# Image-Processing-Systems-Laboratory/DeepInPainting

Hardware: AMD Instinct MI355X
Metric: train images/sec at 256x256, batch 8/GPU, 1/2/4/8 MI355X; IPSR layer ms (higher is better)
Workload: dtype f32; 1 GPU; BASELINE config 2: 256x256 synthetic images, 128x128 centre mask (M=256 of N=1024 feature positions), batch 8/GPU, fp32, full IPSR training step; global_batch=8, parallelism=dp1, dropout=True, conv_math=fp32, vgg16=seeded random init (no pretrained weights offline)

## Files before the change

deepinpainting_amd/csrc/winograd.hip:

```cpp
#include <type_traits>

#include "ipsr_common.h"

namespace ipsr {

typedef float f32x16 __attribute__((ext_vector_type(16)));
typedef const __attribute__((address_space(1))) void* gptr_t;
typedef __attribute__((address_space(3))) void* lptr_t;

constexpr int WG_BM = 128, WG_BN = 128, WG_BK = 16, WG_NBUF = 4, WG_THREADS = 256;

struct WinoSplit {
    int nsplit, sps, xi_split, nsplit_t, sps_t;
    int nxi = 36;
    __host__ __device__ int slabs() const { return xi_split >= nxi ? nsplit : (xi_split <= 0 ? nsplit_t : (nsplit > nsplit_t ? nsplit : nsplit_t)); }
    __host__ __device__ int of(int xi) const { return xi < xi_split ? nsplit : nsplit_t; }
    __host__ __device__ int head_xi() const { return xi_split < nxi ? xi_split : nxi; }
    __host__ int workgroups(int tiles_per_xi) const { return tiles_per_xi * (head_xi() * nsplit + (nxi - head_xi()) * nsplit_t); }
};

__device__ __forceinline__ void wino_load_sum(const float* __restrict__ M, const WinoSplit sp, size_t plane, size_t off, float m[6][6])
{
#pragma unroll
    for (int i = 0; i < 6; ++i)
// ... 1321 lines not shown
            if (oy < Ho && ox < Wo) st1(yp, (size_t)oy * Wo + ox, o[i][j]);
        }
}

constexpr int W5R_TILES = 64;
template <typename TOUT>
__global__ void __launch_bounds__(256) wino5_output_rows_kernel(const float* __restrict__ Mo, WinoSplit split, int B, int K, int Kp, int nh, int nw,
                                                                int TY, int TX, int Tp, TOUT* __restrict__ y)
{
    __shared__ float blk[W5R_TILES][101];
    __shared__ int org_y[W5R_TILES], org_x[W5R_TILES], org_b[W5R_TILES];
    const int tl = threadIdx.x & 63, ph = threadIdx.x >> 6, ey = ph >> 1, ex = ph & 1;
    const int t0 = blockIdx.x * W5R_TILES, t = t0 + tl, k = blockIdx.y;
    const int T = B * TY * TX;
    if (t < T) {
        float m[6][6], o[5][5];
        wino_load_sum(Mo, split, (size_t)Kp * Tp, (size_t)(ph * K + k) * Tp + t, m);
        wino_at5_2d(m, o);
#pragma unroll
        for (int i = 0; i < 5; ++i)
#pragma unroll
            for (int j = 0; j < 5; ++j) blk[tl][(2 * i - ey + 1) * 10 + (2 * j - ex + 1)] = o[i][j];
        if (ph == 0) {
            const int b = t / (TY * TX), rem = t - b * TY * TX;
            const int ty = rem / TX, tx = rem - ty * TX;
            org_b[tl] = b; org_y[tl] = 10 * ty - 1; org_x[tl] = 10 * tx - 1;
        }
    }
    __syncthreads();
    const int Hy = 2 * nh, Wy = 2 * nw;
    const int ntile = min(W5R_TILES, T - t0);
    for (int e = threadIdx.x; e < 10 * 10 * W5R_TILES; e += 256) {
        const int r = e / (10 * W5R_TILES), xs = e - r * (10 * W5R_TILES);
        const int tile = xs / 10, c = xs - tile * 10;
        if (tile >= ntile) continue;
        const int fy = org_y[tile] + r, fx = org_x[tile] + c;
        if (fy < 0 || fy >= Hy || fx < 0 || fx >= Wy) continue;
        st1(y + ((size_t)org_b[tile] * K + k) * (size_t)Hy * Wy, (size_t)fy * Wy + fx, blk[tile][r * 10 + c]);
    }
}

template <int MODE, typename TIN>
__global__ void __launch_bounds__(256) wino_wrw_tile5_kernel(const TIN* __restrict__ dy, int B, int K, int Ho, int Wo, int TY, int TX,
                                                             int Tp, int Kp, void* __restrict__ Et)
{
    __shared__ __attribute__((aligned(16))) unsigned char smem[op_smem_bytes<true, MODE>()];
    const OpIdx ix = op_index<true, MODE>(false);
    const int t = ix.t, k = ix.c, T = B * TY * TX;
    const bool live = t < T && k < K;
    int b = 0, ty = 0, tx = 0;
    if (live) { b = t / (TY * TX); const int rem = t - b * TY * TX; ty = rem / TX; tx = rem - ty * TX; }
    const TIN* dp = dy + ((size_t)b * K + (live ? k : 0)) * Ho * Wo;
    float e[5][5];
#pragma unroll
    for (int i = 0; i < 5; ++i)
#pragma unroll
        for (int j = 0; j < 5; ++j) {
            const int yy = 5 * ty + i, xx = 5 * tx + j;
            e[i][j] = (live && yy < Ho && xx < Wo) ? ld1(dp, (size_t)yy * Wo + xx) : 0.0f;
        }
    float w[6][5], v[6][6];
#pragma unroll
    for (int j = 0; j < 5; ++j) {
        const float col[5] = {e[0][j], e[1][j], e[2][j], e[3][j], e[4][j]};
        float o[6];
        wino_g5(col, o);
#pragma unroll
        for (int i = 0; i < 6; ++i) w[i][j] = o[i];
    }
#pragma unroll
    for (int i = 0; i < 6; ++i) wino_g5(w[i], v[i]);
    op_emit<true, MODE>(smem, v, ix, Et, Kp, Tp);
}

__global__ void __launch_bounds__(256) wino_wrw_output2_kernel(const float* __restrict__ Mw, WinoSplit split, int Kc, int Cf, int Kp, int Cp,
                                                               float* __restrict__ dW)
{
    const int cf = blockIdx.x * 256 + threadIdx.x, kc = blockIdx.y, ph = blockIdx.z;
    if (cf >= Cf) return;
    float m[6][6], w[2][6], o[2][2];
    wino_load_sum(Mw, split, (size_t)Kp * Cp, (size_t)kc * Cp + (size_t)ph * Cf + cf, m);
#pragma unroll
    for (int j = 0; j < 6; ++j) {
        const float col[6] = {m[0][j], m[1][j], m[2][j], m[3][j], m[4][j], m[5][j]};
        float r2[2];
        wino_at2(col, r2);
        w[0][j] = r2[0]; w[1][j] = r2[1];
    }
    wino_at2(w[0], o[0]);
    wino_at2(w[1], o[1]);
    const int ey = ph >> 1, ex = ph & 1;
    float* dst = dW + ((size_t)kc * Cf + cf) * 16;
#pragma unroll
    for (int a = 0; a < 2; ++a)
#pragma unroll
        for (int b = 0; b < 2; ++b) dst[(2 * a + ey) * 4 + 2 * b + ex] = o[a][b];
}

struct S2Plan { int TY, TX, T, Tp, Kp, Cp, red; WinoSplit sp; size_t a_floats, b_floats, m_floats, total_bytes; };

static int s2_plan(int mode, int B, int Kc, int Cf, int nh, int nw, S2Plan* p, int math)
{
    if (mode < 0 || mode > 2) return fail(IPSR_ERR_INVALID, "4x4 stride-2 winograd: mode %d", mode);
    p->TY = mode == 1 ? (nh + 5) / 5 : (nh + 4) / 5;
    p->TX = mode == 1 ? (nw + 5) / 5 : (nw + 4) / 5;
    p->T = B * p->TY * p->TX;
    p->Tp = (p->T + WG_BN - 1) / WG_BN * WG_BN;
    size_t m1;
    if (mode == 2) {
        p->Kp = wino_rows_padded(Kc, math);
        p->Cp = (4 * Cf + WG_BN - 1) / WG_BN * WG_BN;
        p->red = p->Tp;
        p->a_floats = (size_t)36 * p->Tp * p->Kp * 3 / 2;
        p->b_floats = (size_t)36 * p->Tp * p->Cp * 3 / 2;
        m1 = (size_t)36 * p->Kp * p->Cp;
        p->sp = wino_choose_split(36 * wino_row_tiles(p->Kp) * (p->Cp / WG_BN), p->Tp / WG_BK, m1 * 4);
    } else {
        p->red = mode == 0 ? 4 * Cf : Kc;
        if (p->red % WG_BK != 0)
            return fail(IPSR_ERR_UNSUPPORTED, "4x4 stride-2 winograd: reduction length %d is not a multiple of %d", p->red, WG_BK);
        const int prod = mode == 0 ? Kc : 4 * Cf;
        p->Kp = wino_rows_padded(prod, math);
        p->Cp = p->red;
        p->a_floats = (size_t)36 * p->red * p->Kp * 3 / 2;
        p->b_floats = (size_t)36 * p->red * p->Tp * 3 / 2;
        m1 = (size_t)36 * p->Kp * p->Tp;
        p->sp = wino_choose_split(36 * wino_row_tiles(p->Kp) * (p->Tp / WG_BN), p->red / WG_BK, m1 * 4);
    }
    p->m_floats = m1 * p->sp.slabs();
    p->total_bytes = align_up(p->a_floats * 4, 256) + align_up(p->b_floats * 4, 256) + align_up(p->m_floats * 4, 256) + 256;
    return IPSR_OK;
}

size_t winograd_s2_ws_bytes(int mode, int B, int Kc, int Cf, int nh, int nw)
{
    S2Plan p, q;
    if (s2_plan(mode, B, Kc, Cf, nh, nw, &p, -1) != IPSR_OK || s2_plan(mode, B, Kc, Cf, nh, nw, &q, 0) != IPSR_OK) return 0;
    return p.total_bytes > q.total_bytes ? p.total_bytes : q.total_bytes;
}

int launch_winograd_s2(int mode, const void* a, const void* b2, void* out, int B, int Kc, int Cf, int nh, int nw,
                       void* ws, size_t ws_bytes, hipStream_t st, ConvArith ar = ConvArith{0, false, false})
{
    S2Plan p;
    if (int rc = s2_plan(mode, B, Kc, Cf, nh, nw, &p, ar.math)) return rc;
    if (ws_bytes < p.total_bytes) return fail(IPSR_ERR_WORKSPACE, "4x4 stride-2 winograd: workspace %zu < %zu", ws_bytes, p.total_bytes);
    if (!arith_ok(ar)) return fail(IPSR_ERR_INVALID, "4x4 stride-2 winograd: arithmetic %d", ar.math);
    if (ar.math && ((mode == 0 && Cf % 8 != 0) || (mode == 1 && (Cf % SPLIT_ROWS != 0 || p.Kp != 4 * Cf || Kc % 8 != 0)))) ar.math = 0;
    Carver cv(ws, ws_bytes);
    float* A = cv.take<float>(p.a_floats);
    float* Bv = cv.take<float>(p.b_floats);
    float* Mo = cv.take<float>(p.m_floats);
    const int remap = !debug_option(1);
    if (mode == 0 || mode == 1) {
        const float* w = static_cast<const float*>(b2);
        if (ar.math == 0) {
            if (mode == 0) wino52_filter_kernel<<<dim3(cdiv(p.Kp, 256), Cf), 256, 0, st>>>(w, Kc, Cf, p.Kp, 0, A);
            else wino52_filter_kernel<<<dim3(cdiv(Cf + (p.Kp - 4 * Cf), 256), Kc), 256, 0, st>>>(w, Kc, Cf, p.Kp, 1, A);
        } else {
            const dim3 fg = mode == 0 ? dim3(p.Kp / SPLIT_ROWS, Cf / 8) : dim3(Cf / SPLIT_ROWS, Kc / 8);
            if (ar.math == 2) wino52_filter_split_kernel<2><<<fg, 256, 0, st>>>(w, Kc, Cf, p.Kp, mode, reinterpret_cast<unsigned short*>(A));
            else wino52_filter_split_kernel<3><<<fg, 256, 0, st>>>(w, Kc, Cf, p.Kp, mode, reinterpret_cast<unsigned short*>(A));
        }
        with_mode(ar.math, [&](auto M) {
            constexpr int MODE = decltype(M)::value;
            with_type(ar.in_bf16, [&](auto* tag) {
                using T = ELEM_T(tag);
                if (mode == 0) wino5_window_kernel<2, false, MODE, T><<<op_grid(false, MODE, p.Tp, p.red), 256, 0, st>>>(static_cast<const T*>(a), B, Cf, 2 * nh, 2 * nw, 4, p.TY, p.TX, p.Tp, 0, Bv, remap);
                else wino5_window_kernel<1, false, MODE, T><<<op_grid(false, MODE, p.Tp, p.red), 256, 0, st>>>(static_cast<const T*>(a), B, Kc, nh, nw, 1, p.TY, p.TX, p.Tp, 0, Bv, remap);
            });
        });
        if (int rc = check_launch("wino5_window_kernel")) return rc;
        launch_wino_gemm(ar.math, A, Bv, p.red, p.Kp, p.Tp, p.sp, Mo, st, 72.0 * p.red * (mode == 0 ? Kc : 4 * Cf) * p.T);
        if (int rc = check_launch("wino_gemm_kernel")) return rc;
        with_type(ar.out_bf16, [&](auto* tag) {
            using T = ELEM_T(tag);
            if (mode == 0) wino5_output_kernel<T><<<dim3(cdiv(p.T, 256), Kc), 256, 0, st>>>(Mo, p.sp, B, Kc, p.Kp, nh, nw, p.TY, p.TX, p.Tp, static_cast<T*>(out));
            else wino5_output_rows_kernel<T><<<dim3(cdiv(p.T, W5R_TILES), Cf), 256, 0, st>>>(Mo, p.sp, B, Cf, p.Kp, nh, nw, p.TY, p.TX, p.Tp, static_cast<T*>(out));
        });
        return check_launch("wino5_output_kernel");
    }
    with_mode(ar.math, [&](auto M) {
        constexpr int MODE = decltype(M)::value;
        with_type(ar.in_bf16, [&](auto* tag) {
            using T = ELEM_T(tag);
            wino_wrw_tile5_kernel<MODE, T><<<op_grid(true, MODE, p.Tp, p.Kp), 256, 0, st>>>(static_cast<const T*>(b2), B, Kc, nh, nw, p.TY, p.TX, p.Tp, p.Kp, A);
            wino5_window_kernel<2, true, MODE, T><<<op_grid(true, MODE, p.Tp, p.Cp), 256, 0, st>>>(static_cast<const T*>(a), B, Cf, 2 * nh, 2 * nw, 4, p.TY, p.TX, p.Tp, p.Cp, Bv, 0);
        });
    });
    if (int rc = check_launch("wino5_window_kernel")) return rc;
    launch_wino_gemm(ar.math, A, Bv, p.Tp, p.Kp, p.Cp, p.sp, Mo, st, 72.0 * p.T * Kc * 4 * Cf);
    if (int rc = check_launch("wino_gemm_kernel")) return rc;
    wino_wrw_output2_kernel<<<dim3(cdiv(Cf, 256), Kc, 4), 256, 0, st>>>(Mo, p.sp, Kc, Cf, p.Kp, p.Cp, static_cast<float*>(out));
    return check_launch("wino_wrw_output2_kernel");
}

typedef float f32x4v __attribute__((ext_vector_type(4)));


__global__ void __launch_bounds__(256) sm_to_cn_kernel(const float* __restrict__ x, int B, int C, int HW, int Tp, float* __restrict__ out)
{
    const int n = blockIdx.x * 256 + threadIdx.x, c = blockIdx.y;
    if (n >= Tp) return;
    float v = 0.0f;
    if (n < B * HW) { const int b = n / HW, p = n - b * HW; v = x[((size_t)b * C + c) * HW + p]; }
    out[(size_t)c * Tp + n] = v;
}

__global__ void __launch_bounds__(256) sm_to_nc_kernel(const float* __restrict__ x, int B, int C, int HW, float* __restrict__ out)
{
    const int c = blockIdx.x * 256 + threadIdx.x, n = blockIdx.y;
    if (c >= C) return;
    float v = 0.0f;
    if (n < B * HW) { const int b = n / HW, p = n - b * HW; v = x[((size_t)b * C + c) * HW + p]; }
    out[(size_t)n * C + c] = v;
}

__device__ __forceinline__ float sm_tap(const float* __restrict__ f, int B, int C, int Hf, int Wf, int Ho, int Wo, int k, int st, int pad, int dil,
                                        int n, int col)
{
    if (n >= B * Ho * Wo) return 0.0f;
    const int kk = k * k;
    const int c = col / kk, t = col - c * kk, r = t / k, q = t - r * k;
    const int b = n / (Ho * Wo), o = n - b * Ho * Wo, oy = o / Wo, ox = o - oy * Wo;
    const int fy = oy * st - pad + r * dil, fx = ox * st - pad + q * dil;
    return ((unsigned)fy < (unsigned)Hf && (unsigned)fx < (unsigned)Wf) ? f[(((size_t)b * C + c) * Hf + fy) * Wf + fx] : 0.0f;
}

__global__ void __launch_bounds__(256) sm_im2col_nt_kernel(const float* __restrict__ f, int B, int C, int Hf, int Wf, int Ho, int Wo,
                                                           int k, int st, int pad, int dil, float* __restrict__ out)
{
    const int col = blockIdx.x * 256 + threadIdx.x, n = blockIdx.y;
    const int ncol = C * k * k;
    if (col >= ncol) return;
    out[(size_t)n * ncol + col] = sm_tap(f, B, C, Hf, Wf, Ho, Wo, k, st, pad, dil, n, col);
}

__global__ void __launch_bounds__(256) sm_im2col_cn_kernel(const float* __restrict__ f, int B, int C, int Hf, int Wf, int Ho, int Wo,
                                                           int k, int st, int pad, int dil, int Tp, float* __restrict__ out)
{
    const int n = blockIdx.x * 256 + threadIdx.x, col = blockIdx.y;
    if (n >= Tp) return;
    out[(size_t)col * Tp + n] = sm_tap(f, B, C, Hf, Wf, Ho, Wo, k, st, pad, dil, n, col);
}

__global__ void __launch_bounds__(256) sm_col2im_kernel(const float* __restrict__ M, int nslab, size_t slab_stride, int B, int C, int Hf, int Wf,
                                                        int Ho, int Wo, int k, int st, int pad, int dil, int Tp, float* __restrict__ out)
{
    const size_t idx = (size_t)blockIdx.x * 256 + threadIdx.x;
    const size_t total = (size_t)B * C * Hf * Wf;
    if (idx >= total) return;
    const int fx = (int)(idx % Wf), fy = (int)((idx / Wf) % Hf), c = (int)((idx / ((size_t)Wf * Hf)) % C), b = (int)(idx / ((size_t)Wf * Hf * C));
    float acc = 0.0f;
    for (int r = 0; r < k; ++r) {
        const int ny = fy + pad - r * dil;
        if (ny < 0 || ny % st) continue;
        const int oy = ny / st;
        if (oy >= Ho) continue;
        for (int q = 0; q < k; ++q) {
            const int nx = fx + pad - q * dil;
            if (nx < 0 || nx % st) continue;
            const int ox = nx / st;
            if (ox >= Wo) continue;
            const size_t off = (size_t)(c * k * k + r * k + q) * Tp + ((size_t)b * Ho + oy) * Wo + ox;
            for (int sl = 0; sl < nslab; ++sl) acc += M[(size_t)sl * slab_stride + off];
        }
    }
    out[idx] = acc;
}

__global__ void __launch_bounds__(256) sm_sum_to_nchw_kernel(const float* __restrict__ Y, int nslab, size_t slab_stride, int B, int R, int HW, int Tp,
                                                             float* __restrict__ out)
{
    const size_t idx = (size_t)blockIdx.x * 256 + threadIdx.x;
    if (idx >= (size_t)B * R * HW) return;
    const int o = (int)(idx % HW), r = (int)((idx / HW) % R), b = (int)(idx / ((size_t)HW * R));
    const size_t off = (size_t)r * Tp + (size_t)b * HW + o;
    float acc = 0.0f;
    for (int sl = 0; sl < nslab; ++sl) acc += Y[(size_t)sl * slab_stride + off];
    out[idx] = acc;
}

template <int NB>
__device__ __forceinline__ void sm_reduce4(f32x16 (&acc)[NB], float* lds, int wave, int lane)
{
    if (wave > 0) {
#pragma unroll
        for (int nb = 0; nb < NB; ++nb)
#pragma unroll
            for (int e = 0; e < 16; ++e) lds[(((wave - 1) * NB + nb) * 16 + e) * 64 + lane] = acc[nb][e];
    }
    __syncthreads();
    if (wave == 0) {
#pragma unroll
        for (int w = 0; w < 3; ++w)
#pragma unroll
            for (int nb = 0; nb < NB; ++nb)
#pragma unroll
                for (int e = 0; e < 16; ++e) acc[nb][e] += lds[((w * NB + nb) * 16 + e) * 64 + lane];
    }
    __syncthreads();
}

template <int NB>
__global__ void __launch_bounds__(256) sm_data_kernel(const float* __restrict__ Wm, const float* __restrict__ In, int R, int Q, int Tp, int rows_per_wave,
                                                      float* __restrict__ Mcol)
{
    __shared__ float red[3 * NB * 16 * 64];
    const int lane = threadIdx.x & 63, wave = __builtin_amdgcn_readfirstlane(threadIdx.x >> 6), m = lane & 31, h = lane >> 5;
    const int q0 = blockIdx.x * 128, n0 = blockIdx.z * (32 * NB);
    const int ra = min(R, (blockIdx.y * 4 + wave) * rows_per_wave), rb = min(R, ra + rows_per_wave);
    f32x16 acc[4][NB];
#pragma unroll
    for (int j = 0; j < 4; ++j)
#pragma unroll
        for (int nb = 0; nb < NB; ++nb)
#pragma unroll
            for (int e = 0; e < 16; ++e) acc[j][nb][e] = 0.0f;
    const float* wp = Wm + (size_t)(ra + h) * Q + q0 + 4 * m;
    const float* ip = In + (size_t)(ra + h) * Tp + n0 + m;
    constexpr int U = NB == 1 ? 8 : (NB == 2 ? 4 : 2);
    for (int r = ra; r < rb; r += 2 * U) {
        f32x4v a[U];
        float bv[U][NB];
#pragma unroll
        for (int u = 0; u < U; ++u) {
            const bool ok = r + 2 * u < rb;
            a[u] = ok ? *reinterpret_cast<const f32x4v*>(wp + (size_t)2 * u * Q) : f32x4v{0.0f, 0.0f, 0.0f, 0.0f};
#pragma unroll
            for (int nb = 0; nb < NB; ++nb) bv[u][nb] = ok ? ip[(size_t)2 * u * Tp + 32 * nb] : 0.0f;
        }
#pragma unroll
        for (int u = 0; u < U; ++u)
#pragma unroll
            for (int j = 0; j < 4; ++j)
#pragma unroll
                for (int nb = 0; nb < NB; ++nb) acc[j][nb] = __builtin_amdgcn_mfma_f32_32x32x2f32(a[u][j], bv[u][nb], acc[j][nb], 0, 0, 0);
        wp += (size_t)2 * U * Q;
        ip += (size_t)2 * U * Tp;
    }
    float* out = Mcol + (size_t)blockIdx.y * Q * Tp;
#pragma unroll
    for (int j = 0; j < 4; ++j) {
        sm_reduce4<NB>(acc[j], red, wave, lane);
        if (wave == 0) {
#pragma unroll
            for (int nb = 0; nb < NB; ++nb)
#pragma unroll
                for (int e = 0; e < 16; ++e) {
                    const int row = (e & 3) + 8 * (e >> 2) + 4 * h;
                    out[(size_t)(q0 + 4 * row + j) * Tp + n0 + 32 * nb + m] = acc[j][nb][e];
                }
        }
    }
}

template <int NB>
__global__ void __launch_bounds__(256) sm_fwd_kernel(const float* __restrict__ Wm, const float* __restrict__ Xc, int R, int Q, int Tp, int cols_per_wave,
                                                     float* __restrict__ Y)
{
    __shared__ float red[3 * NB * 16 * 64];
    const int lane = threadIdx.x & 63, wave = __builtin_amdgcn_readfirstlane(threadIdx.x >> 6), m = lane & 31, h = lane >> 5;
    const int r0 = blockIdx.x * 32, n0 = blockIdx.z * (32 * NB);
    const int qa = min(Q, (blockIdx.y * 4 + wave) * cols_per_wave), qb = min(Q, qa + cols_per_wave);
    f32x16 acc[NB];
#pragma unroll
    for (int nb = 0; nb < NB; ++nb)
#pragma unroll
        for (int e = 0; e < 16; ++e) acc[nb][e] = 0.0f;
    const float* wp = Wm + (size_t)(r0 + m) * Q + qa + 4 * h;
    const float* xp = Xc + (size_t)(qa + 4 * h) * Tp + n0 + m;
    constexpr int U = 4;
    for (int q = qa; q < qb; q += 8 * U) {
        f32x4v a[U];
        float bv[U][4][NB];
#pragma unroll
        for (int u = 0; u < U; ++u) {
            const bool ok = q + 8 * u < qb;
            a[u] = ok ? *reinterpret_cast<const f32x4v*>(wp + 8 * u) : f32x4v{0.0f, 0.0f, 0.0f, 0.0f};
#pragma unroll
            for (int j = 0; j < 4; ++j)
#pragma unroll
                for (int nb = 0; nb < NB; ++nb) bv[u][j][nb] = ok ? xp[(size_t)(8 * u + j) * Tp + 32 * nb] : 0.0f;
        }
#pragma unroll
        for (int u = 0; u < U; ++u)
#pragma unroll
            for (int j = 0; j < 4; ++j)
#pragma unroll
                for (int nb = 0; nb < NB; ++nb) acc[nb] = __builtin_amdgcn_mfma_f32_32x32x2f32(a[u][j], bv[u][j][nb], acc[nb], 0, 0, 0);
        wp += 8 * U;
        xp += (size_t)8 * U * Tp;
    }
    sm_reduce4<NB>(acc, red, wave, lane);
    if (wave == 0) {
        float* out = Y + (size_t)blockIdx.y * R * Tp;
#pragma unroll
        for (int nb = 0; nb < NB; ++nb)
#pragma unroll
            for (int e = 0; e < 16; ++e) {
                const int row = (e & 3) + 8 * (e >> 2) + 4 * h;
                out[(size_t)(r0 + row) * Tp + n0 + 32 * nb + m] = acc[nb][e];
            }
    }
}

__global__ void __launch_bounds__(64) sm_wrw_kernel(const float* __restrict__ Ct, const float* __restrict__ Vt, int R, int Q, int Pp, float* __restrict__ dW)
{
    const int lane = threadIdx.x, m = lane & 31, h = lane >> 5;
    const int q0 = blockIdx.x * 128, r0 = blockIdx.y * 32;
    f32x16 acc[4];
#pragma unroll
    for (int j = 0; j < 4; ++j)
#pragma unroll
        for (int e = 0; e < 16; ++e) acc[j][e] = 0.0f;
    const float* cp = Ct + (size_t)h * R + r0 + m;
    const float* vp = Vt + (size_t)h * Q + q0 + 4 * m;
    constexpr int U = 4;
    for (int p = 0; p < Pp; p += 2 * U) {
        float av[U];
        f32x4v b[U];
#pragma unroll
        for (int u = 0; u < U; ++u) {
            const bool ok = p + 2 * u < Pp;
            av[u] = ok ? cp[(size_t)2 * u * R] : 0.0f;
            b[u] = ok ? *reinterpret_cast<const f32x4v*>(vp + (size_t)2 * u * Q) : f32x4v{0.0f, 0.0f, 0.0f, 0.0f};
        }
#pragma unroll
        for (int u = 0; u < U; ++u)
#pragma unroll
            for (int j = 0; j < 4; ++j) acc[j] = __builtin_amdgcn_mfma_f32_32x32x2f32(av[u], b[u][j], acc[j], 0, 0, 0);
        cp += (size_t)2 * U * R;
        vp += (size_t)2 * U * Q;
    }
#pragma unroll
    for (int e = 0; e < 16; ++e) {
        const int row = (e & 3) + 8 * (e >> 2) + 4 * h;
        *reinterpret_cast<f32x4v*>(dW + (size_t)(r0 + row) * Q + q0 + 4 * m) = f32x4v{acc[0][e], acc[1][e], acc[2][e], acc[3][e]};
    }
}

struct SmPlan { int P, Tp, Pp, Q, nb, ngroups, nslab, per_slab; size_t a_floats, b_floats, m_floats, total_bytes; };

static int sm_plan(int op, int B, int R, int Cq, int Ho, int Wo, int Hf, int Wf, int k, int st, int pad, int dil, SmPlan* p)
{
    if (op < 0 || op > 2) return fail(IPSR_ERR_INVALID, "small-map convolution: op %d", op);
    if (k < 1 || k > 4 || st < 1 || st > 2 || dil < 1 || pad < 0) return fail(IPSR_ERR_UNSUPPORTED, "small-map convolution: k%d s%d p%d d%d", k, st, pad, dil);
    if (Ho != (Hf + 2 * pad - dil * (k - 1) - 1) / st + 1 || Wo != (Wf + 2 * pad - dil * (k - 1) - 1) / st + 1)
        return fail(IPSR_ERR_INVALID, "small-map convolution: %dx%d is not the output grid of %dx%d under k%d s%d p%d d%d", Ho, Wo, Hf, Wf, k, st, pad, dil);
    p->P = B * Ho * Wo;
    p->Q = Cq * k * k;
    if (p->Q % 128 != 0) return fail(IPSR_ERR_UNSUPPORTED, "small-map convolution: %d x %d taps is not a multiple of 128", Cq, k * k);
    if (R % 32 != 0) return fail(IPSR_ERR_UNSUPPORTED, "small-map convolution: %d weight rows are not a multiple of 32", R);
    if (p->P > 1024) return fail(IPSR_ERR_UNSUPPORTED, "small-map convolution: %d positions (made for <= 1024)", p->P);
    const int blocks = (p->P + 31) / 32;
    p->nb = blocks >= 4 ? 4 : (blocks == 3 ? 4 : blocks);
    if (op == 0 && p->nb == 4) p->nb = 2;
    p->ngroups = (blocks + p->nb - 1) / p->nb;
    p->Tp = p->ngroups * p->nb * 32;
    p->Pp = (p->P + 1) & ~1;
    p->a_floats = p->b_floats = p->m_floats = 0;
    p->nslab = 1; p->per_slab = 0;
    const size_t w_bytes = (size_t)R * p->Q * 4;
    if (op == 0) {
        const int qb = p->Q / 128;
        const size_t slab_bytes = (size_t)p->Q * p->Tp * 4;
        const int cap = (int)std::max<size_t>(1, w_bytes / slab_bytes);
        int ns = std::max(1, std::min({R / 64, cap, (256 + qb * p->ngroups - 1) / (qb * p->ngroups)}));
        p->per_slab = (((R + 4 * ns - 1) / (4 * ns)) + 1) & ~1;
        p->nslab = (R + 4 * p->per_slab - 1) / (4 * p->per_slab);
        p->b_floats = (size_t)R * p->Tp;
        p->m_floats = (size_t)p->nslab * p->Q * p->Tp;
    } else if (op == 2) {
        const int rb = R / 32;
        const size_t slab_bytes = (size_t)R * p->Tp * 4;
        const int cap = (int)std::max<size_t>(1, w_bytes / slab_bytes);
        int ns = std::max(1, std::min({p->Q / 256, cap, (256 + rb * p->ngroups - 1) / (rb * p->ngroups)}));
        p->per_slab = (((p->Q + 4 * ns - 1) / (4 * ns)) + 7) & ~7;
        p->nslab = (p->Q + 4 * p->per_slab - 1) / (4 * p->per_slab);
        p->b_floats = (size_t)p->Q * p->Tp;
        p->m_floats = (size_t)p->nslab * R * p->Tp;
    } else {
        p->a_floats = (size_t)p->Pp * R;
        p->b_floats = (size_t)p->Pp * p->Q;
    }
    p->total_bytes = align_up(p->a_floats * 4, 256) + align_up(p->b_floats * 4, 256) + align_up(p->m_floats * 4, 256) + 256;
    return IPSR_OK;
}

size_t smallmap_ws_bytes(int op, int B, int R, int Cq, int Ho, int Wo, int Hf, int Wf, int k, int st, int pad, int dil)
{
    SmPlan p;
    if (sm_plan(op, B, R, Cq, Ho, Wo, Hf, Wf, k, st, pad, dil, &p) != IPSR_OK) return 0;
    return p.total_bytes;
}

int launch_smallmap(int op, const float* a, const float* b2, float* out, int B, int R, int Cq, int Ho, int Wo, int Hf, int Wf,
                    int k, int st_, int pad, int dil, void* ws, size_t ws_bytes, hipStream_t st)
{
    SmPlan p;
    if (int rc = sm_plan(op, B, R, Cq, Ho, Wo, Hf, Wf, k, st_, pad, dil, &p)) return rc;
    if (ws_bytes < p.total_bytes) return fail(IPSR_ERR_WORKSPACE, "small-map convolution: workspace %zu < %zu", ws_bytes, p.total_bytes);
    Carver cv(ws, ws_bytes);
    float* A = cv.take<float>(p.a_floats);
    float* Bv = cv.take<float>(p.b_floats);
    float* Mo = cv.take<float>(p.m_floats);
    if (op == 0) {
        sm_to_cn_kernel<<<dim3(cdiv(p.Tp, 256), R), 256, 0, st>>>(a, B, R, Ho * Wo, p.Tp, Bv);
        const dim3 grid(p.Q / 128, p.nslab, p.ngroups);
        if (p.nb == 1) sm_data_kernel<1><<<grid, 256, 0, st>>>(b2, Bv, R, p.Q, p.Tp, p.per_slab, Mo);
        else sm_data_kernel<2><<<grid, 256, 0, st>>>(b2, Bv, R, p.Q, p.Tp, p.per_slab, Mo);
        if (int rc = check_launch("sm_data_kernel")) return rc;
        const size_t total = (size_t)B * Cq * Hf * Wf;
        sm_col2im_kernel<<<(unsigned)((total + 255) / 256), 256, 0, st>>>(Mo, p.nslab, (size_t)p.Q * p.Tp, B, Cq, Hf, Wf, Ho, Wo, k, st_, pad, dil, p.Tp, out);
        return check_launch("sm_col2im_kernel");
    }
    if (op == 2) {
        sm_im2col_cn_kernel<<<dim3(cdiv(p.Tp, 256), p.Q), 256, 0, st>>>(a, B, Cq, Hf, Wf, Ho, Wo, k, st_, pad, dil, p.Tp, Bv);
        const dim3 grid(R / 32, p.nslab, p.ngroups);
        if (p.nb == 1) sm_fwd_kernel<1><<<grid, 256, 0, st>>>(b2, Bv, R, p.Q, p.Tp, p.per_slab, Mo);
        else if (p.nb == 2) sm_fwd_kernel<2><<<grid, 256, 0, st>>>(b2, Bv, R, p.Q, p.Tp, p.per_slab, Mo);
        else sm_fwd_kernel<4><<<grid, 256, 0, st>>>(b2, Bv, R, p.Q, p.Tp, p.per_slab, Mo);
        if (int rc = check_launch("sm_fwd_kernel")) return rc;
        const size_t total = (size_t)B * R * Ho * Wo;
        sm_sum_to_nchw_kernel<<<(unsigned)((total + 255) / 256), 256, 0, st>>>(Mo, p.nslab, (size_t)R * p.Tp, B, R, Ho * Wo, p.Tp, out);
        return check_launch("sm_sum_to_nchw_kernel");
    }
    sm_to_nc_kernel<<<dim3(cdiv(R, 256), p.Pp), 256, 0, st>>>(a, B, R, Ho * Wo, A);
    sm_im2col_nt_kernel<<<dim3(cdiv(p.Q, 256), p.Pp), 256, 0, st>>>(b2, B, Cq, Hf, Wf, Ho, Wo, k, st_, pad, dil, Bv);
    sm_wrw_kernel<<<dim3(p.Q / 128, R / 32), 64, 0, st>>>(A, Bv, R, p.Q, p.Pp, out);
    return check_launch("sm_wrw_kernel");
}

}

using namespace ipsr;

extern "C" {

int ipsr_debug_force_wino_split(int nsplit, int xi_split, int nsplit_t)
{
    if (nsplit == 0 && xi_split == 0 && nsplit_t == 0) { g_force_split[0] = g_force_split[1] = g_force_split[2] = 0; return IPSR_OK; }
    if (nsplit < 1 || nsplit_t < 1 || xi_split < 1 || xi_split > 36) return fail(IPSR_ERR_INVALID, "ipsr_debug_force_wino_split: bad split %d,%d,%d", nsplit, xi_split, nsplit_t);
    g_force_split[0] = nsplit; g_force_split[1] = xi_split; g_force_split[2] = nsplit_t;
    return IPSR_OK;
}

int ipsr_wino_gemm_split(int rows, int cols, int reduction, int* out5)
{
    if (!out5 || rows < 1 || cols < 1 || reduction < 1 || rows % WG_BM || cols % WG_BN || reduction % WG_BK)
        return fail(IPSR_ERR_INVALID, "ipsr_wino_gemm_split: rows / cols must be multiples of 128 and the reduction of 16");
    const WinoSplit sp = wino_choose_split(36 * (rows / WG_BM) * (cols / WG_BN), reduction / WG_BK, (size_t)36 * rows * cols * 4);
    out5[0] = sp.nsplit; out5[1] = sp.sps; out5[2] = sp.xi_split; out5[3] = sp.nsplit_t; out5[4] = sp.sps_t;
    return IPSR_OK;
}

size_t ipsr_conv3x3_winograd_workspace_bytes(int op, int B, int Cin, int H, int W, int Cout)
{
    if (op < 0 || op > 3 || B < 1 || Cin < 1 || Cout < 1 || H < 1 || W < 1) return 0;
    const bool fwd = op == 0 || op == 2;
    return winograd_ws_bytes(B, fwd ? Cin : Cout, fwd ? Cout : Cin, H, W);
}

static int arith_from(const char* who, int math, int io, ConvArith* ar)
{
    if ((math != 0 && math != 2 && math != 3) || io < 0 || io > 3)
        return fail(IPSR_ERR_INVALID, "%s: math %d (0 = fp32 MFMA, 2 = split bf16 x3, 3 = split bf16 x6) / io %d (bit 0: bf16 activations in, bit 1: out)", who, math, io);
    ar->math = math; ar->in_bf16 = (io & 1) != 0; ar->out_bf16 = (io & 2) != 0;
    return IPSR_OK;
}

int ipsr_conv3x3_winograd_mp(int op, const void* in, const float* weight, const float* bias, int epilogue, float* filter_cache,
                             int filter_cache_valid, void* out, int B, int Cin, int H, int W, int Cout, int math, int io,
                             void* ws, size_t ws_bytes, void* stream)
{
    if (!in || !weight || !out || !ws) return fail(IPSR_ERR_INVALID, "ipsr_conv3x3_winograd: null pointer");
    if (op < 0 || op > 3 || B < 1 || Cin < 1 || Cout < 1 || H < 1 || W < 1) return fail(IPSR_ERR_INVALID, "ipsr_conv3x3_winograd: bad argument");
    if ((reinterpret_cast<uintptr_t>(ws) & 15u) || (reinterpret_cast<uintptr_t>(out) & 15u) || (reinterpret_cast<uintptr_t>(filter_cache) & 15u))
        return fail(IPSR_ERR_INVALID, "ipsr_conv3x3_winograd: out / workspace / filter_cache must be 16-byte aligned");
    ConvArith ar;
    if (int rc = arith_from("ipsr_conv3x3_winograd_mp", math, io, &ar)) return rc;
    if (reinterpret_cast<uintptr_t>(in) & (ar.in_bf16 ? 7u : 15u))
        return fail(IPSR_ERR_INVALID, "ipsr_conv3x3_winograd: in must be aligned to four elements");
    hipStream_t st = static_cast<hipStream_t>(stream);
    switch (op) {
        case 0:
            return launch_winograd(in, weight, out, B, Cin, Cout, H, W, 9, (long)Cin * 9, 0, ws, ws_bytes, st, bias, epilogue, filter_cache, filter_cache_valid, ar);
        case 1:
            return launch_winograd(in, weight, out, B, Cout, Cin, H, W, (long)Cin * 9, 9, 1, ws, ws_bytes, st, bias, epilogue, filter_cache, filter_cache_valid, ar);
        case 2:
            return launch_winograd(in, weight, out, B, Cin, Cout, H, W, (long)Cout * 9, 9, 1, ws, ws_bytes, st, bias, epilogue, filter_cache, filter_cache_valid, ar);
        default:
            return launch_winograd(in, weight, out, B, Cout, Cin, H, W, 9, (long)Cout * 9, 0, ws, ws_bytes, st, bias, epilogue, filter_cache, filter_cache_valid, ar);
    }
}

int ipsr_conv3x3_winograd(int op, const float* in, const float* weight, float* out, int B, int Cin, int H, int W, int Cout,
                          void* ws, size_t ws_bytes, void* stream)
{
    return ipsr_conv3x3_winograd_mp(op, in, weight, nullptr, 0, nullptr, 0, out, B, Cin, H, W, Cout, 0, 0, ws, ws_bytes, stream);
}

size_t ipsr_conv3x3_winograd_filter_floats(int op, int Cin, int Cout)
{
    if (op < 0 || op > 3 || Cin < 1 || Cout < 1) return 0;
    const bool fwd = op == 0 || op == 2;
    return winograd_filter_floats(fwd ? Cin : Cout, fwd ? Cout : Cin);
}

int ipsr_conv3x3_winograd_ex(int op, const float* in, const float* weight, const float* bias, int epilogue, float* filter_cache,
                             int filter_cache_valid, float* out, int B, int Cin, int H, int W, int Cout,
                             void* ws, size_t ws_bytes, void* stream)
{
    return ipsr_conv3x3_winograd_mp(op, in, weight, bias, epilogue, filter_cache, filter_cache_valid, out, B, Cin, H, W, Cout, 0, 0, ws, ws_bytes, stream);
}

size_t ipsr_conv4x4_winograd_workspace_bytes(int geom, int mode, int B, int Cin, int H, int W, int Cout)
{
    if (geom < 0 || geom > 1 || mode < 0 || mode > 2 || B < 1 || Cin < 1 || Cout < 1 || H < 2 || W < 2) return 0;
    return winograd_dil_ws_bytes(geom, mode, B, Cin, H, W, Cout);
}

int ipsr_conv4x4_winograd_mp(int geom, int mode, const void* a, const void* b, void* out, int B, int Cin, int H, int W, int Cout,
                             int math, int io, void* ws, size_t ws_bytes, void* stream)
{
    if (!a || !b || !out || !ws) return fail(IPSR_ERR_INVALID, "ipsr_conv4x4_winograd: null pointer");
    if (geom < 0 || geom > 1 || mode < 0 || mode > 2 || B < 1 || Cin < 1 || Cout < 1 || H < 2 || W < 2)
        return fail(IPSR_ERR_INVALID, "ipsr_conv4x4_winograd: bad argument");
    if ((reinterpret_cast<uintptr_t>(ws) & 15u) || (reinterpret_cast<uintptr_t>(out) & 15u))
        return fail(IPSR_ERR_INVALID, "ipsr_conv4x4_winograd: out / workspace must be 16-byte aligned");
    ConvArith ar;
    if (int rc = arith_from("ipsr_conv4x4_winograd_mp", math, io, &ar)) return rc;
    return launch_winograd_dil(geom, mode, a, b, out, B, Cin, H, W, Cout, ws, ws_bytes, static_cast<hipStream_t>(stream), ar);
}

int ipsr_conv4x4_winograd(int geom, int mode, const float* a, const float* b, float* out, int B, int Cin, int H, int W, int Cout,
                          void* ws, size_t ws_bytes, void* stream)
{
    return ipsr_conv4x4_winograd_mp(geom, mode, a, b, out, B, Cin, H, W, Cout, 0, 0, ws, ws_bytes, stream);
}

size_t ipsr_conv4x4_dilated_winograd_workspace_bytes(int mode, int B, int Cin, int H, int W, int Cout)
{
    return ipsr_conv4x4_winograd_workspace_bytes(0, mode, B, Cin, H, W, Cout);
}

int ipsr_conv4x4_dilated_winograd(int mode, const float* a, const float* b, float* out, int B, int Cin, int H, int W, int Cout,
                                  void* ws, size_t ws_bytes, void* stream)
{
    return ipsr_conv4x4_winograd(0, mode, a, b, out, B, Cin, H, W, Cout, ws, ws_bytes, stream);
}

size_t ipsr_conv4x4s2_winograd_workspace_bytes(int mode, int B, int Kc, int Cf, int nh, int nw)
{
    if (mode < 0 || mode > 2 || B < 1 || Kc < 1 || Cf < 1 || nh < 1 || nw < 1) return 0;
    return winograd_s2_ws_bytes(mode, B, Kc, Cf, nh, nw);
}

int ipsr_conv4x4s2_winograd_mp(int mode, const void* a, const void* b, void* out, int B, int Kc, int Cf, int nh, int nw,
                               int math, int io, void* ws, size_t ws_bytes, void* stream)
{
    if (!a || !b || !out || !ws) return fail(IPSR_ERR_INVALID, "ipsr_conv4x4s2_winograd: null pointer");
    if (mode < 0 || mode > 2 || B < 1 || Kc < 1 || Cf < 1 || nh < 1 || nw < 1) return fail(IPSR_ERR_INVALID, "ipsr_conv4x4s2_winograd: bad argument");
    if ((reinterpret_cast<uintptr_t>(ws) & 15u) || (reinterpret_cast<uintptr_t>(out) & 15u))
        return fail(IPSR_ERR_INVALID, "ipsr_conv4x4s2_winograd: out / workspace must be 16-byte aligned");
    if (mode != 2 && (reinterpret_cast<uintptr_t>(b) & 15u))
        return fail(IPSR_ERR_INVALID, "ipsr_conv4x4s2_winograd: the weight must be 16-byte aligned");
    ConvArith ar;
    if (int rc = arith_from("ipsr_conv4x4s2_winograd_mp", math, io, &ar)) return rc;
    return launch_winograd_s2(mode, a, b, out, B, Kc, Cf, nh, nw, ws, ws_bytes, static_cast<hipStream_t>(stream), ar);
}

int ipsr_conv4x4s2_winograd(int mode, const float* a, const float* b, float* out, int B, int Kc, int Cf, int nh, int nw,
                            void* ws, size_t ws_bytes, void* stream)
{
    return ipsr_conv4x4s2_winograd_mp(mode, a, b, out, B, Kc, Cf, nh, nw, 0, 0, ws, ws_bytes, stream);
}

size_t ipsr_conv_smallmap_workspace_bytes(int op, int B, int R, int Cq, int Ho, int Wo, int Hf, int Wf, int k, int stride, int pad, int dil)
{
    if (B < 1 || R < 1 || Cq < 1 || Ho < 1 || Wo < 1 || Hf < 1 || Wf < 1) return 0;
    return smallmap_ws_bytes(op, B, R, Cq, Ho, Wo, Hf, Wf, k, stride, pad, dil);
}

int ipsr_conv_smallmap(int op, const float* a, const float* b, float* out, int B, int R, int Cq, int Ho, int Wo, int Hf, int Wf,
                       int k, int stride, int pad, int dil, void* ws, size_t ws_bytes, void* stream)
{
    if (!a || !b || !out || !ws) return fail(IPSR_ERR_INVALID, "ipsr_conv_smallmap: null pointer");
    if (B < 1 || R < 1 || Cq < 1 || Ho < 1 || Wo < 1 || Hf < 1 || Wf < 1) return fail(IPSR_ERR_INVALID, "ipsr_conv_smallmap: bad argument");
    if ((reinterpret_cast<uintptr_t>(ws) & 15u) || (reinterpret_cast<uintptr_t>(out) & 15u) || (reinterpret_cast<uintptr_t>(a) & 15u) ||
        (reinterpret_cast<uintptr_t>(b) & 15u))
        return fail(IPSR_ERR_INVALID, "ipsr_conv_smallmap: operands / workspace must be 16-byte aligned");
    return launch_smallmap(op, a, b, out, B, R, Cq, Ho, Wo, Hf, Wf, k, stride, pad, dil, ws, ws_bytes, static_cast<hipStream_t>(stream));
}

size_t ipsr_conv3x3_winograd_wrw_workspace_bytes(int transposed, int B, int Cin, int H, int W, int Cout)
{
    if (B < 1 || Cin < 1 || Cout < 1 || H < 1 || W < 1) return 0;
    return transposed ? winograd_wrw_ws_bytes(B, Cin, Cout, H, W) : winograd_wrw_ws_bytes(B, Cout, Cin, H, W);
}

int ipsr_conv3x3_winograd_wrw_mp(int transposed, const void* x, const void* dy, float* dw, int B, int Cin, int H, int W, int Cout,
                                 int math, int io, void* ws, size_t ws_bytes, void* stream)
{
    if (!x || !dy || !dw || !ws) return fail(IPSR_ERR_INVALID, "ipsr_conv3x3_winograd_wrw: null pointer");
    if (B < 1 || Cin < 1 || Cout < 1 || H < 1 || W < 1) return fail(IPSR_ERR_INVALID, "ipsr_conv3x3_winograd_wrw: bad argument");
    if (reinterpret_cast<uintptr_t>(ws) & 15u) return fail(IPSR_ERR_INVALID, "ipsr_conv3x3_winograd_wrw: workspace must be 16-byte aligned");
    ConvArith ar;
    if (int rc = arith_from("ipsr_conv3x3_winograd_wrw_mp", math, io, &ar)) return rc;
    hipStream_t st = static_cast<hipStream_t>(stream);
    if (transposed) return launch_winograd_wrw(x, dy, dw, B, Cin, Cout, H, W, ws, ws_bytes, st, ar);
    return launch_winograd_wrw(dy, x, dw, B, Cout, Cin, H, W, ws, ws_bytes, st, ar);
}

int ipsr_conv3x3_winograd_wrw(int transposed, const float* x, const float* dy, float* dw, int B, int Cin, int H, int W, int Cout,
                              void* ws, size_t ws_bytes, void* stream)
{
    return ipsr_conv3x3_winograd_wrw_mp(transposed, x, dy, dw, B, Cin, H, W, Cout, 0, 0, ws, ws_bytes, stream);
}

}
```

Measured before the change: 343.6 images/sec.

## Fuse im2col and layout transposes into small-map conv GEMM kernels via gather addressing

The small-map convolution GEMM kernels (data-grad, forward, weight-grad) now compute im2col and NCHW-to-CN gather offsets themselves and read the original tensors directly. This skips the separate transpose and im2col kernels along with their workspace writes and reads. The cost is extra integer address math, scattered uncoalesced loads, per-iteration tap masking, and an LDS position table in the weight-grad kernel. The path is gated on size limits that keep offsets within 32 bits, and on a debug option.

```diff
diff --git a/deepinpainting_amd/csrc/winograd.hip b/deepinpainting_amd/csrc/winograd.hip
--- a/deepinpainting_amd/csrc/winograd.hip
+++ b/deepinpainting_amd/csrc/winograd.hip
@@ -1647,9 +1647,55 @@
     __syncthreads();
 }
 
+struct SmGeom { int B, C, Hf, Wf, Ho, Wo, k, st, pad, dil; unsigned mkk, mk; };
+constexpr unsigned SM_OFFSET = (1u << 28) - 1;
+
+__device__ __forceinline__ unsigned sm_column(const SmGeom& g, int col)
+{
+    const int c = (int)__umulhi(2u * (unsigned)col, g.mkk);
+    const int t = col - c * g.k * g.k;
+    const int r = (int)__umulhi(2u * (unsigned)t, g.mk), q = t - r * g.k;
+    return (unsigned)t << 28 | 4u * (unsigned)((c * g.Hf + r * g.dil) * g.Wf + q * g.dil);
+}
+
+__device__ __forceinline__ int sm_position(const SmGeom& g, int n, unsigned& taps)
+{
+    taps = 0;
+    if (n >= g.B * g.Ho * g.Wo) return 0;
+    const int b = n / (g.Ho * g.Wo), o = n - b * g.Ho * g.Wo, oy = o / g.Wo, ox = o - oy * g.Wo;
+    const int fy = oy * g.st - g.pad, fx = ox * g.st - g.pad;
+    unsigned cols = 0;
+    for (int q = 0; q < g.k; ++q) cols |= (unsigned)((unsigned)(fx + q * g.dil) < (unsigned)g.Wf) << q;
+    for (int r = 0; r < g.k; ++r)
+        if ((unsigned)(fy + r * g.dil) < (unsigned)g.Hf) taps |= cols << (r * g.k);
+    return 4 * ((b * g.C * g.Hf + fy) * g.Wf + fx);
+}
+
 template <int NB>
+__device__ __forceinline__ void sm_fwd_columns(const SmGeom& g, int q, int lane, const int (&pos)[NB], const unsigned (&taps)[NB],
+                                               unsigned (&off)[4][4][NB], unsigned (&keep)[NB])
+{
+    const unsigned mine = sm_column(g, q + (lane & 31));
+    const int h = lane >> 5;
+#pragma unroll
+    for (int nb = 0; nb < NB; ++nb) keep[nb] = 0;
+#pragma unroll
+    for (int u = 0; u < 4; ++u)
+#pragma unroll
+        for (int j = 0; j < 4; ++j) {
+            const unsigned w = __shfl(mine, 8 * u + 4 * h + j);
+#pragma unroll
+            for (int nb = 0; nb < NB; ++nb) {
+                const unsigned in = (taps[nb] >> (w >> 28)) & 1u;
+                off[u][j][nb] = in ? ((unsigned)pos[nb] + w) & SM_OFFSET : 0u;
+                keep[nb] |= in << (4 * u + j);
+            }
+        }
+}
+
+template <int NB, bool GATHER>
 __global__ void __launch_bounds__(256) sm_data_kernel(const float* __restrict__ Wm, const float* __restrict__ In, int R, int Q, int Tp, int rows_per_wave,
-                                                      float* __restrict__ Mcol)
+                                                      int B, int HW, float* __restrict__ Mcol)
 {
     __shared__ float red[3 * NB * 16 * 64];
     const int lane = threadIdx.x & 63, wave = __builtin_amdgcn_readfirstlane(threadIdx.x >> 6), m = lane & 31, h = lane >> 5;
@@ -1664,6 +1710,17 @@
             for (int e = 0; e < 16; ++e) acc[j][nb][e] = 0.0f;
     const float* wp = Wm + (size_t)(ra + h) * Q + q0 + 4 * m;
     const float* ip = In + (size_t)(ra + h) * Tp + n0 + m;
+    unsigned go[NB];
+    bool live[NB];
+    if constexpr (GATHER) {
+#pragma unroll
+        for (int nb = 0; nb < NB; ++nb) {
+            const int n = n0 + 32 * nb + m;
+            live[nb] = n < B * HW;
+            const int b = live[nb] ? n / HW : 0, p = live[nb] ? n - b * HW : 0;
+            go[nb] = 4u * (unsigned)((b * R + ra + h) * HW + p);
+        }
+    }
     constexpr int U = NB == 1 ? 8 : (NB == 2 ? 4 : 2);
     for (int r = ra; r < rb; r += 2 * U) {
         f32x4v a[U];
@@ -1673,7 +1730,14 @@
             const bool ok = r + 2 * u < rb;
             a[u] = ok ? *reinterpret_cast<const f32x4v*>(wp + (size_t)2 * u * Q) : f32x4v{0.0f, 0.0f, 0.0f, 0.0f};
 #pragma unroll
-            for (int nb = 0; nb < NB; ++nb) bv[u][nb] = ok ? ip[(size_t)2 * u * Tp + 32 * nb] : 0.0f;
+            for (int nb = 0; nb < NB; ++nb) {
+                if constexpr (GATHER) {
+                    const float v = ok ? *reinterpret_cast<const float*>(reinterpret_cast<const char*>(In) + (go[nb] + 8u * (unsigned)(u * HW))) : 0.0f;
+                    bv[u][nb] = live[nb] ? v : 0.0f;
+                } else {
+                    bv[u][nb] = ok ? ip[(size_t)2 * u * Tp + 32 * nb] : 0.0f;
+                }
+            }
         }
 #pragma unroll
         for (int u = 0; u < U; ++u)
@@ -1683,6 +1747,10 @@
                 for (int nb = 0; nb < NB; ++nb) acc[j][nb] = __builtin_amdgcn_mfma_f32_32x32x2f32(a[u][j], bv[u][nb], acc[j][nb], 0, 0, 0);
         wp += (size_t)2 * U * Q;
         ip += (size_t)2 * U * Tp;
+        if constexpr (GATHER) {
+#pragma unroll
+            for (int nb = 0; nb < NB; ++nb) go[nb] += 8u * (unsigned)(U * HW);
+        }
     }
     float* out = Mcol + (size_t)blockIdx.y * Q * Tp;
 #pragma unroll
@@ -1700,9 +1768,9 @@
     }
 }
 
-template <int NB>
+template <int NB, bool GATHER>
 __global__ void __launch_bounds__(256) sm_fwd_kernel(const float* __restrict__ Wm, const float* __restrict__ Xc, int R, int Q, int Tp, int cols_per_wave,
-                                                     float* __restrict__ Y)
+                                                     SmGeom g, float* __restrict__ Y)
 {
     __shared__ float red[3 * NB * 16 * 64];
     const int lane = threadIdx.x & 63, wave = __builtin_amdgcn_readfirstlane(threadIdx.x >> 6), m = lane & 31, h = lane >> 5;
@@ -1716,17 +1784,41 @@
     const float* wp = Wm + (size_t)(r0 + m) * Q + qa + 4 * h;
     const float* xp = Xc + (size_t)(qa + 4 * h) * Tp + n0 + m;
     constexpr int U = 4;
+    int pos[NB];
+    unsigned taps[NB], off[U][4][NB], keep[NB];
+    const bool same_taps = (8 * U) % (g.k * g.k) == 0;
+    const unsigned step = 4u * (unsigned)((8 * U) / (g.k * g.k) * g.Hf * g.Wf);
     for (int q = qa; q < qb; q += 8 * U) {
         f32x4v a[U];
         float bv[U][4][NB];
-#pragma unroll
-        for (int u = 0; u < U; ++u) {
-            const bool ok = q + 8 * u < qb;
-            a[u] = ok ? *reinterpret_cast<const f32x4v*>(wp + 8 * u) : f32x4v{0.0f, 0.0f, 0.0f, 0.0f};
-#pragma unroll
-            for (int j = 0; j < 4; ++j)
-#pragma unroll
-                for (int nb = 0; nb < NB; ++nb) bv[u][j][nb] = ok ? xp[(size_t)(8 * u + j) * Tp + 32 * nb] : 0.0f;
+        if constexpr (GATHER) {
+#pragma unroll
+            for (int u = 0; u < U; ++u)
+                a[u] = q + 8 * u < qb ? *reinterpret_cast<const f32x4v*>(wp + 8 * u) : f32x4v{0.0f, 0.0f, 0.0f, 0.0f};
+            if (q == qa) {
+#pragma unroll
+                for (int nb = 0; nb < NB; ++nb) pos[nb] = sm_position(g, n0 + 32 * nb + m, taps[nb]);
+            }
+            if (q == qa || !same_taps) sm_fwd_columns<NB>(g, q, lane, pos, taps, off, keep);
+#pragma unroll
+            for (int u = 0; u < U; ++u)
+#pragma unroll
+                for (int j = 0; j < 4; ++j)
+#pragma unroll
+                    for (int nb = 0; nb < NB; ++nb) {
+                        const float v = q + 8 * u < qb ? *reinterpret_cast<const float*>(reinterpret_cast<const char*>(Xc) + off[u][j][nb]) : 0.0f;
+                        bv[u][j][nb] = (keep[nb] >> (4 * u + j)) & 1u ? v : 0.0f;
+                    }
+        } else {
+#pragma unroll
+            for (int u = 0; u < U; ++u) {
+                const bool ok = q + 8 * u < qb;
+                a[u] = ok ? *reinterpret_cast<const f32x4v*>(wp + 8 * u) : f32x4v{0.0f, 0.0f, 0.0f, 0.0f};
+#pragma unroll
+                for (int j = 0; j < 4; ++j)
+#pragma unroll
+                    for (int nb = 0; nb < NB; ++nb) bv[u][j][nb] = ok ? xp[(size_t)(8 * u + j) * Tp + 32 * nb] : 0.0f;
+            }
         }
 #pragma unroll
         for (int u = 0; u < U; ++u)
@@ -1736,6 +1828,16 @@
                 for (int nb = 0; nb < NB; ++nb) acc[nb] = __builtin_amdgcn_mfma_f32_32x32x2f32(a[u][j], bv[u][j][nb], acc[nb], 0, 0, 0);
         wp += 8 * U;
         xp += (size_t)8 * U * Tp;
+        if constexpr (GATHER) {
+            if (same_taps) {
+#pragma unroll
+                for (int u = 0; u < U; ++u)
+#pragma unroll
+                    for (int j = 0; j < 4; ++j)
+#pragma unroll
+                        for (int nb = 0; nb < NB; ++nb) off[u][j][nb] += step;
+            }
+        }
     }
     sm_reduce4<NB>(acc, red, wave, lane);
     if (wave == 0) {
@@ -1750,10 +1852,28 @@
     }
 }
 
-__global__ void __launch_bounds__(64) sm_wrw_kernel(const float* __restrict__ Ct, const float* __restrict__ Vt, int R, int Q, int Pp, float* __restrict__ dW)
+template <bool GATHER>
+__global__ void __launch_bounds__(64) sm_wrw_kernel(const float* __restrict__ Ct, const float* __restrict__ Vt, int R, int Q, int Pp, SmGeom g,
+                                                    float* __restrict__ dW)
 {
     const int lane = threadIdx.x, m = lane & 31, h = lane >> 5;
     const int q0 = blockIdx.x * 128, r0 = blockIdx.y * 32;
+    extern __shared__ int4 ptab[];
+    unsigned col[4], a_lane = 0;
+    if constexpr (GATHER) {
+        const int HW = g.Ho * g.Wo;
+        for (int n = lane; n < Pp; n += 64) {
+            unsigned taps;
+            const int pos = sm_position(g, n, taps);
+            const bool live = n < g.B * HW;
+            const int b = live ? n / HW : 0;
+            ptab[n] = int4{pos, (int)taps, live ? 4 * (b * (R - 1) * HW + n) : 0, live ? 1 : 0};
+        }
+#pragma unroll
+        for (int j = 0; j < 4; ++j) col[j] = sm_column(g, q0 + 4 * m + j);
+        a_lane = 4u * (unsigned)((r0 + m) * HW);
+        __syncthreads();
+    }
     f32x16 acc[4];
 #pragma unroll
     for (int j = 0; j < 4; ++j)
@@ -1768,8 +1888,24 @@
 #pragma unroll
         for (int u = 0; u < U; ++u) {
             const bool ok = p + 2 * u < Pp;
-            av[u] = ok ? cp[(size_t)2 * u * R] : 0.0f;
-            b[u] = ok ? *reinterpret_cast<const f32x4v*>(vp + (size_t)2 * u * Q) : f32x4v{0.0f, 0.0f, 0.0f, 0.0f};
+            if constexpr (GATHER) {
+                av[u] = 0.0f;
+                b[u] = f32x4v{0.0f, 0.0f, 0.0f, 0.0f};
+                if (ok) {
+                    const int4 e = ptab[p + 2 * u + h];
+                    const float a = *reinterpret_cast<const float*>(reinterpret_cast<const char*>(Ct) + ((unsigned)e.z + a_lane));
+                    av[u] = e.w ? a : 0.0f;
+#pragma unroll
+                    for (int j = 0; j < 4; ++j) {
+                        const bool in = ((unsigned)e.y >> (col[j] >> 28)) & 1u;
+                        const float v = *reinterpret_cast<const float*>(reinterpret_cast<const char*>(Vt) + (in ? ((unsigned)e.x + col[j]) & SM_OFFSET : 0u));
+                        b[u][j] = in ? v : 0.0f;
+                    }
+                }
+            } else {
+                av[u] = ok ? cp[(size_t)2 * u * R] : 0.0f;
+                b[u] = ok ? *reinterpret_cast<const f32x4v*>(vp + (size_t)2 * u * Q) : f32x4v{0.0f, 0.0f, 0.0f, 0.0f};
+            }
         }
 #pragma unroll
         for (int u = 0; u < U; ++u)
@@ -1850,30 +1986,50 @@
     float* A = cv.take<float>(p.a_floats);
     float* Bv = cv.take<float>(p.b_floats);
     float* Mo = cv.take<float>(p.m_floats);
+    const int form = debug_option(2);
+    const size_t reach = (size_t)B * Cq * Hf * Wf + (size_t)(k - 1) * dil * (Wf + 1);
+    const bool gather = form != 1 && (size_t)B * R * Ho * Wo < (1u << 26) && reach < (1u << 26) && p.Q < (1 << 26) && (op != 1 || p.P <= 32 || form == 2);
+    const SmGeom g = {B, Cq, Hf, Wf, Ho, Wo, k, st_, pad, dil, (1u << 31) / (k * k) + 1, (1u << 31) / k + 1};
     if (op == 0) {
-        sm_to_cn_kernel<<<dim3(cdiv(p.Tp, 256), R), 256, 0, st>>>(a, B, R, Ho * Wo, p.Tp, Bv);
         const dim3 grid(p.Q / 128, p.nslab, p.ngroups);
-        if (p.nb == 1) sm_data_kernel<1><<<grid, 256, 0, st>>>(b2, Bv, R, p.Q, p.Tp, p.per_slab, Mo);
-        else sm_data_kernel<2><<<grid, 256, 0, st>>>(b2, Bv, R, p.Q, p.Tp, p.per_slab, Mo);
+        if (gather) {
+            if (p.nb == 1) sm_data_kernel<1, true><<<grid, 256, 0, st>>>(b2, a, R, p.Q, p.Tp, p.per_slab, B, Ho * Wo, Mo);
+            else sm_data_kernel<2, true><<<grid, 256, 0, st>>>(b2, a, R, p.Q, p.Tp, p.per_slab, B, Ho * Wo, Mo);
+        } else {
+            sm_to_cn_kernel<<<dim3(cdiv(p.Tp, 256), R), 256, 0, st>>>(a, B, R, Ho * Wo, p.Tp, Bv);
+            if (p.nb == 1) sm_data_kernel<1, false><<<grid, 256, 0, st>>>(b2, Bv, R, p.Q, p.Tp, p.per_slab, B, Ho * Wo, Mo);
+            else sm_data_kernel<2, false><<<grid, 256, 0, st>>>(b2, Bv, R, p.Q, p.Tp, p.per_slab, B, Ho * Wo, Mo);
+        }
         if (int rc = check_launch("sm_data_kernel")) return rc;
         const size_t total = (size_t)B * Cq * Hf * Wf;
         sm_col2im_kernel<<<(unsigned)((total + 255) / 256), 256, 0, st>>>(Mo, p.nslab, (size_t)p.Q * p.Tp, B, Cq, Hf, Wf, Ho, Wo, k, st_, pad, dil, p.Tp, out);
         return check_launch("sm_col2im_kernel");
     }
     if (op == 2) {
-        sm_im2col_cn_kernel<<<dim3(cdiv(p.Tp, 256), p.Q), 256, 0, st>>>(a, B, Cq, Hf, Wf, Ho, Wo, k, st_, pad, dil, p.Tp, Bv);
         const dim3 grid(R / 32, p.nslab, p.ngroups);
-        if (p.nb == 1) sm_fwd_kernel<1><<<grid, 256, 0, st>>>(b2, Bv, R, p.Q, p.Tp, p.per_slab, Mo);
-        else if (p.nb == 2) sm_fwd_kernel<2><<<grid, 256, 0, st>>>(b2, Bv, R, p.Q, p.Tp, p.per_slab, Mo);
-        else sm_fwd_kernel<4><<<grid, 256, 0, st>>>(b2, Bv, R, p.Q, p.Tp, p.per_slab, Mo);
+        if (gather) {
+            if (p.nb == 1) sm_fwd_kernel<1, true><<<grid, 256, 0, st>>>(b2, a, R, p.Q, p.Tp, p.per_slab, g, Mo);
+            else if (p.nb == 2) sm_fwd_kernel<2, true><<<grid, 256, 0, st>>>(b2, a, R, p.Q, p.Tp, p.per_slab, g, Mo);
+            else sm_fwd_kernel<4, true><<<grid, 256, 0, st>>>(b2, a, R, p.Q, p.Tp, p.per_slab, g, Mo);
+        } else {
+            sm_im2col_cn_kernel<<<dim3(cdiv(p.Tp, 256), p.Q), 256, 0, st>>>(a, B, Cq, Hf, Wf, Ho, Wo, k, st_, pad, dil, p.Tp, Bv);
+            if (p.nb == 1) sm_fwd_kernel<1, false><<<grid, 256, 0, st>>>(b2, Bv, R, p.Q, p.Tp, p.per_slab, g, Mo);
+            else if (p.nb == 2) sm_fwd_kernel<2, false><<<grid, 256, 0, st>>>(b2, Bv, R, p.Q, p.Tp, p.per_slab, g, Mo);
+            else sm_fwd_kernel<4, false><<<grid, 256, 0, st>>>(b2, Bv, R, p.Q, p.Tp, p.per_slab, g, Mo);
+        }
         if (int rc = check_launch("sm_fwd_kernel")) return rc;
         const size_t total = (size_t)B * R * Ho * Wo;
         sm_sum_to_nchw_kernel<<<(unsigned)((total + 255) / 256), 256, 0, st>>>(Mo, p.nslab, (size_t)R * p.Tp, B, R, Ho * Wo, p.Tp, out);
         return check_launch("sm_sum_to_nchw_kernel");
     }
-    sm_to_nc_kernel<<<dim3(cdiv(R, 256), p.Pp), 256, 0, st>>>(a, B, R, Ho * Wo, A);
-    sm_im2col_nt_kernel<<<dim3(cdiv(p.Q, 256), p.Pp), 256, 0, st>>>(b2, B, Cq, Hf, Wf, Ho, Wo, k, st_, pad, dil, Bv);
-    sm_wrw_kernel<<<dim3(p.Q / 128, R / 32), 64, 0, st>>>(A, Bv, R, p.Q, p.Pp, out);
+    const dim3 grid(p.Q / 128, R / 32);
+    if (gather) {
+        sm_wrw_kernel<true><<<grid, 64, (size_t)p.Pp * sizeof(int4), st>>>(a, b2, R, p.Q, p.Pp, g, out);
+    } else {
+        sm_to_nc_kernel<<<dim3(cdiv(R, 256), p.Pp), 256, 0, st>>>(a, B, R, Ho * Wo, A);
+        sm_im2col_nt_kernel<<<dim3(cdiv(p.Q, 256), p.Pp), 256, 0, st>>>(b2, B, Cq, Hf, Wf, Ho, Wo, k, st_, pad, dil, Bv);
+        sm_wrw_kernel<false><<<grid, 64, 0, st>>>(A, Bv, R, p.Q, p.Pp, g, out);
+    }
     return check_launch("sm_wrw_kernel");
 }
 
```

After: 344.2 images/sec, median of 2. About the same (+0.2%).
